# xiaoh/sediFoam

Hardware: AMD Instinct MI355X
Metric: particle-DEM-substeps/sec (higher is better)
Workload: dtype f64; 1 GPU; 1M-particle monodisperse Hertz-history packing (FCC bed, d=1mm, 2% overlap), periodic x/z, wall y, gravity + fix fdrag, 50 DEM sub-steps per step; particles_total=1000188, particles_per_gpu=1000188, neighbor_rebuilds_in_run=140, decomposition=single domain

## Files before the change

### sedifoam_amd/csrc/sf_dem.h

```cpp
#pragma once
#include <map>
#include <string>
#include <vector>
#include <cstdint>
#include <string>
#include <vector>

#include "sf_common.h"
#include "sf_physics.h"

namespace sf {

constexpr int kNeighMask = 0x3FFFFFFF;
constexpr int kTouchBit = 0x40000000;
constexpr int kOwnBit = (int)0x80000000;
constexpr int kIdxBits = 25;
constexpr int kIdxMask = (1 << kIdxBits) - 1;
constexpr int kNoShift = 13;
__host__ __device__ __forceinline__ int neigh_index(int word, int roots)
{
  return roots ? (word & kIdxMask) : (word & kNeighMask);
}
__device__ __forceinline__ void shift_to_image(double4& x, const int word, const double (&prd)[3])
{
// ... 62 lines not shown
constexpr int kBlkMask = (1 << kBlkShift) - 1;
__host__ __device__ inline int* header_vote_ptr(double* slot) { return reinterpret_cast<int*>(slot); }
__host__ __device__ inline int header_vote(const double* slot) { return *reinterpret_cast<const int*>(slot); }

struct DemPtrs {
  const double4* xr_in;
  const double4* vm_in;
  const double4* om_in;
  double4* xr_out;
  double4* vm_out;
  double4* om_out;
  double4* force;
  double4* torque;
  int* neigh;
  int* numneigh;
  const double* shear_in;
  double* shear_out;
  double* fdrag;
  double* DuDt;
  double* vOld;
  double* wshear;
  unsigned char* wtouch;
  const double* xhold;
  const int* mask;
  int* flags;
  const int* sendslot[2];
  double* tx[2];
  double* tx_sendbuf;
  const int* bslot;
  double* const* tx_blkptr;
  const size_t* tx_blkcnt;
  const int* tx_hdr_off;
  int* xcd_time;
  const double* tx_blkshift;
  const struct GsSync* gs_sync;
  int* gs_my_sync;
  int* gs_count;
  const unsigned short* nloc;
  const int* tile_first;
  const int* tile_last;
  const int* stage_start;
  const int* stage_idx;
  const double* mbody;
};

struct GsSync {
  int world, rank;
  long long max_ticks;
  int* my_sync;
  int* peer_sync[32];
};
constexpr int kGsStride = 32;

struct StepParams {
  int nlocal, cap, mode;
  int kstep;
  int nslots;
  int roots;
  double prd[3];
  int part, nb;
  int n_lo, n_hi;
  int trig_test;
  int trig_set;
  int trig_add;
  double margin_sq;
  double dt, trigger_sq;
  GranParams gran;
  CoheParams cohe;
  LubParams lub;
  int nwalls;
  int stage_cap;
  int xcd_remap;
  int xcd_first[8], xcd_count[8];
  int xcd_time;
  WallParams wall[kMaxWalls];
  int have_gravity;
  double gacc[3];
  int have_fdrag;
  double carrier_rho;
  int have_nve;
  int use_groups, nve_bit, grav_bit, fdrag_bit, cohe_bit, freeze_bit;
  int post_freeze;
  int tx_fused, tx_nhdr;
  double tx_lo3[3], tx_hi3[3];
  int gs_on, gs_seq, gs_wait;
  int gs_world, gs_rank;
  int tx_n[2];
  double tx_xlo, tx_xhi, tx_shift[2];
};

struct BinGrid {
  double lo[3], inv[3];
  int n[3];
  int stencil;
  int nbins;
  int tile;
  int nt[3];
  int xslow;
  int wrap[3];
};

__host__ __device__ __forceinline__ int bin_key(const BinGrid& g, int cx, int cy, int cz)
{
  if (g.xslow) return cz + g.n[2] * (cy + g.n[1] * cx);
  if (g.tile <= 1) return cx + g.n[0] * (cy + g.n[1] * cz);
  const int T = g.tile;
  const int tx = cx / T, ty = cy / T, tz = cz / T;
  const int lx = cx - tx * T, ly = cy - ty * T, lz = cz - tz * T;
  return ((tx + g.nt[0] * (ty + g.nt[1] * tz)) * T + lz) * T * T + ly * T + lx;
}

__device__ __forceinline__ int block_sum_int_1024(int v)
{
  __shared__ int ws[16];
  for (int off = 32; off > 0; off >>= 1) v += __shfl_down(v, off, 64);
  const int lane = threadIdx.x & 63, w = threadIdx.x >> 6;
  __syncthreads();
  if (lane == 0) ws[w] = v;
  __syncthreads();
  int t = 0;
  if (threadIdx.x == 0)
    for (int k = 0; k < (int)(blockDim.x >> 6); k++) t += ws[k];
  return t;
}

struct RebuildPredictor {
  long long last = 0;
// ... 384 lines not shown
  LubParams lub_{};
  int nwalls_ = 0;
  WallParams walls_[kMaxWalls];
  WallMotion wall_motion_[kMaxWalls];
  long long wall_time_origin_ = 0;
  long long run_base_step_ = 0;
  bool have_gravity_ = false, have_fdrag_ = false, have_nve_ = false;
  std::map<std::string, int> groups_{{"all", 1}};
  bool use_groups_ = false;
  int nve_bit_ = 1, grav_bit_ = 1, fdrag_bit_ = 1, cohe_bit_ = 1, freeze_bit_ = 0;
  int post_freeze_ = 0;
  int new_group_bit(const std::string& name);
  void mark_frozen();
  double gacc_[3] = {0, 0, 0};
  double carrier_rho_ = 0.0;

  DevArray xr_[2], vm_[2], om_[2], force_, torque_;
  DevArray tag_, type_, mask_, foamCpuId_;
  DevArray fdrag_, DuDt_, vOld_, xhold_;
  DevArray extra_;
  int nextra_ = 0;
  unsigned extra_used_ = 0;
  double extra_init_[8] = {0, 0, 0, 0, 0, 0, 0, 0};
  DevArray wshear_, wtouch_;
  DevArray gsrc_, gshift_;
  DevArray neigh_, numneigh_, shear_[2];
  DevArray neigh_old_, numneigh_old_, ptag_;
  int flags_seq_ = 0;
  bool build_flags_clean_ = false;
  int park_rows_ = 0;
  bool hist_in_place_ = false;
  bool hist_in_place_env_ = true;
  bool build_lds_env_ = true;
  bool rank_permute_env_ = true;
  bool ghost_defer_env_ = true;
  int park_margin_env_ = 8;
  bool build_quad_set_ = false;
  int build_quad_env_ = 0;
  bool build_parks_in_lds() const;
  int hist_buf_ = 0;
  bool hist_single_ = true;
  int hist_mode_env_ = 0;
  bool touch_prefetch_ = true;
  int touch_prefetch_env_ = -1;
  bool touch_first_ = false;
  int touch_first_env_ = -1;
  int opt_lpa_ = 0;
  int opt_ghost_free_ = -1;
  bool ghost_free_ = false;
  int nimages_ = -1;
  bool in_run_ = false;
  RebuildPredictor predict_;
  int nt_policy_ = 2, nt_policy_env_ = -1;
  void measure_list();
  ListStats list_stats() const;
  long long list_sampled_ = 0;
  void choose_kernel();
  DevArray nloc_;
  int* tile_tab_ = nullptr;
  size_t tile_alloc_ = 0;
  int* stage_idx_ = nullptr;
  size_t stage_alloc_ = 0;
  int* eoff_ = nullptr;
  size_t eoff_alloc_ = 0;
  int ntiles_ = 0, stage_cap_ = 0;
  bool lds_active_ = false;
  void build_stage_tables();
  DevArray tmp4_, tmpd_, tmpi_;
  DevArray tmp4b_, tmp4c_, tmpi_b_, tmpi_c_, tmpi_d_, fdrag_alt_, DuDt_alt_, vOld_alt_, extra_alt_, wtouch_alt_;
  DevArray keys_, keys_alt_, perm_, perm_alt_, keys64_, keys64_alt_;
  int* cell_start_ = nullptr;
  size_t cell_alloc_ = 0;
  struct CellRowTables {
    int* own_count;
    int* own_first;
    int* ghost_count;
    int* ghost_first;
  };
  CellRowTables cell_row_tables() const
  {
    return {cell_start_, cell_start_ + cell_alloc_, cell_start_ + 2 * cell_alloc_, cell_start_ + 3 * cell_alloc_};
  }
  struct CellRanges {
    static constexpr int stride = 4;
    int* own_start;
    int* own_end;
    int* ghost_start;
    int* ghost_end;
  };
  CellRanges cell_ranges() const { return {cell_start_, cell_start_ + 1, cell_start_ + 2, cell_start_ + 3}; }
  DevArray hist_perm_;
  bool hist_indirect_ = false;
  bool row_tables_ = false;
  int* image_ = nullptr;
  size_t image_rows_ = 0;
  bool uncounted_wraps_ = false;
  void images_fit();
  int* tagmap_ = nullptr;
  size_t tagmap_alloc_ = 0;
  long long order_version_ = 0, tagmap_builds_ = -1;
  struct IoBuf {
    void* p = nullptr;
    size_t n = 0;
  };
  IoBuf io_d_[3], io_i_[2];
  double* io_doubles(int which, size_t n);
// ... 100 lines not shown
```

### sedifoam_amd/csrc/sf_dem.hip

```cpp
#include "sf_dem.h"

#include <algorithm>
#include <atomic>
#include <chrono>
#include <cmath>
#include <cstdlib>
#include <vector>

#include "sf_dem_dispatch.h"
#include "sf_dem_kernels.h"
#include "sf_dem_rebuild.h"
#include "sf_dem_io.h"
#include "sf_env.h"
#include "sf_dem_lds_kernel.h"
#include "sf_list_policy.h"
#include "sf_rigid.h"
#include "sf_roctx.h"
#include "sf_thermo.h"

namespace sf {

std::string& last_error()
{
  static thread_local std::string e;
// ... 57 lines not shown
    fail("Illegal pair_style command");
  p.kn /= nktv2p;
  p.kt /= nktv2p;
  p.beta = (style == 2 && gamman > 0.0) ? hertz_beta(gamman) : 0.0;
  fold_hertz_constants(p);
}

DemEngine::DemEngine()
{
  int ndev = 0;
  hipError_t e = hipGetDeviceCount(&ndev);
  if (e != hipSuccess || ndev == 0)
    fail("sedifoam_amd: no HIP device available (%s) -- this library has no CPU path",
         e == hipSuccess ? "device count 0" : hipGetErrorString(e));
  SF_HIP(hipStreamCreateWithFlags(&own_stream_, hipStreamNonBlocking));
  stream_ = own_stream_;
  SF_HIP(hipMalloc(&own_flags_, sizeof(int) * F_NFLAGS));
  d_flags_ = own_flags_;
  SF_HIP(hipMalloc(&count64_, sizeof(unsigned long long)));
  SF_HIP(hipHostMalloc(&h_flags_, sizeof(int) * F_NFLAGS));
  memset(h_flags_, 0, sizeof(int) * F_NFLAGS);
  SF_HIP(hipMemsetAsync(d_flags_, 0, sizeof(int) * F_NFLAGS, stream_));
  SF_HIP(hipEventCreate(&ev0_));
  SF_HIP(hipEventCreate(&ev1_));
  SF_HIP(hipEventCreateWithFlags(&ev_flags_, hipEventDisableTiming));
  opt_tile_ = env_int("SF_TILE", opt_tile_);
  opt_xcd_remap_ = env_int("SF_XCD_REMAP", opt_xcd_remap_);
  SF_HIP(hipMalloc(&d_xcd_time_, sizeof(int) * 1024));
  SF_HIP(hipHostMalloc(&h_xcd_time_, sizeof(int) * 1024));
  for (int k = 0; k < 512; k++) h_xcd_time_[512 + k] = (k & 63) == 0 ? INT_MAX : 0;
  SF_HIP(hipMemcpyAsync(d_xcd_time_ + 512, h_xcd_time_ + 512, sizeof(int) * 512, hipMemcpyHostToDevice, stream_));
  xcd_auto_ = env_flag("SF_XCD_BALANCE", xcd_auto_);
  if (const char* e = env_str("SF_XCD_WEIGHTS")) {
    double w[8];
    if (sscanf(e, "%lf,%lf,%lf,%lf,%lf,%lf,%lf,%lf", &w[0], &w[1], &w[2], &w[3], &w[4], &w[5], &w[6], &w[7]) == 8) {
      for (int x = 0; x < 8; x++) xcd_weight_[x] = w[x] > 0.0 ? w[x] : 1.0;
      xcd_weighted_ = true;
      xcd_auto_ = false;
    }
  }
  opt_lds_ = env_int("SF_LDS", opt_lds_);
  roots_ = !opt_lds_;
  if ((opt_sub_env_ = env_override("SF_SUB", opt_sub_))) opt_sub_ = std::max(1, opt_sub_);
  hist_mode_env_ = env_int("SF_HIST_COPIES", hist_mode_env_);
  hist_in_place_env_ = env_flag("SF_HIST_IN_PLACE", hist_in_place_env_);
  build_lds_env_ = env_flag("SF_BUILD_LDS", build_lds_env_);
  rank_permute_env_ = env_flag("SF_RANK_PERMUTE", rank_permute_env_);
  build_quad_set_ = env_override("SF_BUILD_QUAD", build_quad_env_);
  ghost_defer_env_ = env_flag("SF_GHOST_DEFER", ghost_defer_env_);
  park_margin_env_ = env_int("SF_PARK_MARGIN", park_margin_env_);
  touch_prefetch_env_ = env_int("SF_TOUCH_PREFETCH", touch_prefetch_env_);
  touch_first_env_ = env_int("SF_TOUCH_FIRST", touch_first_env_);
  nt_policy_env_ = env_int("SF_NT_POLICY", nt_policy_env_);
  opt_lpa_ = env_int("SF_LPA", opt_lpa_);
  opt_ghost_free_ = env_int("SF_GHOST_FREE", opt_ghost_free_);
  predict_.on = env_flag("SF_QUEUE_PREDICT", predict_.on);
  memset(&gran_, 0, sizeof(gran_));
  memset(&cohe_, 0, sizeof(cohe_));
  memset(&lub_, 0, sizeof(lub_));
  per_atom_ = {&xr_[0], &xr_[1], &vm_[0], &vm_[1], &om_[0], &om_[1], &force_, &torque_, &tag_, &type_,
               &mask_, &foamCpuId_, &fdrag_, &DuDt_, &vOld_, &xhold_, &extra_, &wshear_, &wtouch_, &gsrc_, &gshift_,
               &neigh_, &numneigh_, &shear_[0], &shear_[1], &neigh_old_, &numneigh_old_, &ptag_, &tmp4_,
               &tmpd_, &tmpi_, &keys_, &keys_alt_, &perm_, &perm_alt_, &keys64_, &keys64_alt_,
               &sendlist_[0], &sendlist_[1], &leave_, &nloc_, &isb_, &hist_perm_, &bmask_, &tmp4b_, &tmp4c_,
               &tmpi_b_, &tmpi_c_, &tmpi_d_, &fdrag_alt_, &DuDt_alt_, &vOld_alt_, &extra_alt_, &wtouch_alt_};
}

DemEngine::~DemEngine()
{
  if (stream_) (void)hipStreamSynchronize(stream_);
  rigid_release();
  for (DevArray* a : per_atom_) a->release();
  if (d_blkptr_) (void)hipFree(d_blkptr_);
#ifdef SF_EXP_BUILD_PHASE
  {
    unsigned long long h[8] = {0, 0, 0, 0, 0, 0, 0, 0};
    if (hipMemcpyFromSymbol(h, HIP_SYMBOL(g_build_phase), sizeof(h)) == hipSuccess && (h[0] | h[1] | h[3])) {
      const double tot = (double)(h[0] + h[1] + h[2] + h[3] + h[4] + h[5]);
      fprintf(stderr, "[sedifoam_amd] k_build_neigh wave cycles by phase (%d builds): prologue %.3f  walk %.3f  old tags %.3f  "
              "touch-first pass %.3f  second sweep %.3f  counts %.3f  (sum %.3e cycles)\n", (int)nbuilds_, h[0] / tot, h[1] / tot,
              h[5] / tot, h[2] / tot, h[3] / tot, h[4] / tot, tot);
    }
  }
#endif
  if (thermo_vbuf_) (void)hipFree(thermo_vbuf_);
  if (d_xcd_time_) (void)hipFree(d_xcd_time_);
  if (h_xcd_time_) (void)hipHostFree(h_xcd_time_);
  bslot_.release();
  if (cell_start_) (void)hipFree(cell_start_);
  if (tile_tab_) (void)hipFree(tile_tab_);
  if (bsend_list_) (void)hipFree(bsend_list_);
  if (d_bcount_) (void)hipFree(d_bcount_);
  if (h_bcount_) (void)hipHostFree(h_bcount_);
  if (stage_idx_) (void)hipFree(stage_idx_);
  if (eoff_) (void)hipFree(eoff_);
  if (tagmap_) (void)hipFree(tagmap_);
  if (image_) (void)hipFree(image_);
  for (IoBuf& b : io_d_)
    if (b.p) (void)hipFree(b.p);
  for (IoBuf& b : io_i_)
    if (b.p) (void)hipFree(b.p);
  if (sort_tmp_) (void)hipFree(sort_tmp_);
  if (own_flags_) (void)hipFree(own_flags_);
  if (count64_) (void)hipFree(count64_);
  restart_release();
  if (h_flags_) (void)hipHostFree(h_flags_);
// ... 593 lines not shown
  P.wtouch = wtouch_.as<unsigned char>();
  P.xhold = xhold_.as<double>();
  P.mask = mask_.as<int>();
  P.flags = d_flags_;
  P.nloc = nloc_.as<unsigned short>();
  P.tile_first = tile_tab_;
  for (int f = 0; f < 2; f++) {
    P.sendslot[f] = tx_ready_ ? sendslot_.as<int>() + (size_t)f * sendslot_.cap : nullptr;
    P.tx[f] = tx_ptr_[f];
  }
  P.tx_sendbuf = tx_sendbuf_;
  P.bslot = bslot_.as<int>();
  P.tx_blkptr = d_blkptr_ ? d_blkptr_ + (size_t)tx_par_ * kMaxDirs : nullptr;
  static_assert(sizeof(size_t) == sizeof(double*), "the count row of the block table");
  P.tx_blkcnt = d_blkptr_ ? reinterpret_cast<const size_t*>(d_blkptr_ + 2 * (size_t)kMaxDirs) : nullptr;
  P.tx_hdr_off = tx_hdr_off_;
  P.tx_blkshift = nullptr;
  P.gs_sync = nullptr;
  P.gs_my_sync = nullptr;
  P.gs_count = nullptr;
  P.xcd_time = d_xcd_time_;
  P.tile_last = tile_tab_ ? tile_tab_ + tile_alloc_ : nullptr;
  P.stage_start = tile_tab_ ? tile_tab_ + 3 * tile_alloc_ : nullptr;
  P.stage_idx = stage_idx_;
  P.mbody = rigid_rows_.ptr ? rigid_rows_.as<double>() + (size_t)RR_MBODY * cap_ : nullptr;
  return P;
}

StepParams DemEngine::step_params(int mode, int kstep) const
{
  StepParams S;
  memset(&S, 0, sizeof(S));
  S.nlocal = nlocal_;
  S.cap = (int)cap_;
  S.mode = mode;
  S.kstep = kstep;
  S.nslots = M_;
  S.dt = dt_;
  S.trigger_sq = (0.5 * skin_) * (0.5 * skin_);
  S.roots = roots_ ? 1 : 0;
  for (int k = 0; k < 3; k++) S.prd[k] = boxhi_[k] - boxlo_[k];
  S.part = 0;
  S.nb = 0;
  S.trig_test = F_TRIGGER;
  S.trig_set = F_TRIGGER;
  S.trig_add = 0;
  S.margin_sq = 0.0;
  S.gran = gran_;
  S.cohe = cohe_;
  S.lub = lub_;
  S.nwalls = nwalls_;
  S.xcd_remap = opt_xcd_remap_;
  S.stage_cap = stage_cap_;
  const long long steps = (mode == 2 ? nsteps_ : run_base_step_ + kstep + 1) - wall_time_origin_;
  for (int w = 0; w < nwalls_; w++) {
    WallParams W = walls_[w];
    const WallMotion& M = wall_motion_[w];
    if (M.wiggle) {
      const double om = 2.0 * 3.14159265358979323846 / M.period;
      const double arg = om * (double)steps * dt_;
      if (W.dim == M.axis) {
        W.lo = M.lo0 + M.amplitude - M.amplitude * cos(arg);
        W.hi = M.hi0 + M.amplitude - M.amplitude * cos(arg);
      }
      W.vwall[M.axis] = M.amplitude * om * sin(arg);
    } else if (M.shear) {
      if (W.dim == 3 && M.axis != 2) W.vrot = M.vshear;
      else W.vwall[M.axis] = M.vshear;
    }
    S.wall[w] = W;
  }
  S.have_gravity = have_gravity_;
  for (int k = 0; k < 3; k++) S.gacc[k] = gacc_[k];
  S.have_fdrag = have_fdrag_;
  S.carrier_rho = carrier_rho_;
  S.have_nve = have_nve_;
  S.use_groups = use_groups_ ? 1 : 0;
  S.nve_bit = nve_bit_;
  S.grav_bit = grav_bit_;
  S.fdrag_bit = fdrag_bit_;
  S.cohe_bit = cohe_bit_;
  S.freeze_bit = freeze_bit_;
  S.post_freeze = post_freeze_;
  return S;
}

template <int STYLE, bool COHE, bool LUB, bool GS>
static void launch_plain(int lpa, bool tp, int ntp, dim3 grid, int block, hipStream_t s, const DemPtrs& P,
                         const StepParams& S)
{
  auto go = [&](auto lanes, auto policy) {
    constexpr int LPA = decltype(lanes)::value, NTP = decltype(policy)::value;
    if constexpr (LUB && !COHE) k_substep<STYLE, COHE, LUB, LPA, true, NTP, GS><<<grid, block, 0, s>>>(P, S);
    else if (tp || LUB) k_substep<STYLE, COHE, LUB, LPA, true, NTP, GS><<<grid, block, 0, s>>>(P, S);
    else k_substep<STYLE, COHE, LUB, LPA, false, NTP, GS><<<grid, block, 0, s>>>(P, S);
  };
  if (lpa == 4) go(int_c<4>{}, int_c<0>{});
  else if (lpa == 2) go(int_c<2>{}, int_c<0>{});
  else if (GS || ntp == 0) go(int_c<1>{}, int_c<0>{});
  else if constexpr (!GS) {
    if (ntp == 1) go(int_c<1>{}, int_c<1>{});
    else if (ntp == 3) go(int_c<1>{}, int_c<3>{});
    else go(int_c<1>{}, int_c<2>{});
  }
}

template <int STYLE, bool COHE, bool LUB>
static void launch_lds_one(dim3 grid, size_t lds, hipStream_t s, const DemPtrs& P, const StepParams& S)
{
  static size_t granted = 0;
  if (lds > 65536 && lds > granted) {
    SF_HIP(hipFuncSetAttribute(reinterpret_cast<const void*>(&k_substep_lds<STYLE, COHE, LUB>),
                               hipFuncAttributeMaxDynamicSharedMemorySize, 160 * 1024));
    granted = 160 * 1024;
  }
  static const int threads = env_int("SF_LDS_THREADS", 256);
  k_substep_lds<STYLE, COHE, LUB><<<grid, threads, lds, s>>>(P, S);
}

int DemEngine::lanes_per_atom(int nwork) const
{
  if (opt_lpa_ == 1 || opt_lpa_ == 2 || opt_lpa_ == 4) return opt_lpa_;
  if (nwork < 20 * 1024) return 4;
  if (nwork >= 300 * 1024) return 1;
  static const int slots = [] {
    int dev = 0, cus = 256;
    if (hipGetDevice(&dev) == hipSuccess) (void)hipDeviceGetAttribute(&cus, hipDeviceAttributeMultiprocessorCount, dev);
    return cus * 4 * 3;
  }();
  const double r = (double)nwork / 64.0 / (double)slots;
  if (touch_first_) return 0.5 * std::ceil(2.0 * r) <= std::ceil(r) ? 2 : 1;
  return 0.55 * std::ceil(2.0 * r) < std::ceil(r) ? 2 : 1;
}

void DemEngine::launch_thermo_virial(const DemPtrs& P, const StepParams& S)
{
  if (!thermo_vbuf_) SF_HIP(hipMalloc(&thermo_vbuf_, sizeof(double) * 6 * ::sf::thermo_virial_blocks(INT_MAX)));
  thermo_vblocks_ = ::sf::thermo_virial_blocks(nlocal_);
  thermo_virial_launch(P, S, lub_.enabled != 0, thermo_vbuf_, thermo_vblocks_, stream_);
  thermo_vlaunches_++;
}

void DemEngine::substep_empty_rank(int mode, int kstep, bool gs)
{
  if (thermo_virial_on_ && mode != 0) {
// ... 76 lines not shown
      hipEvent_t e;
      SF_HIP(hipEventCreate(&e));
      prof_ev_.push_back(e);
    }
  }
  if (prof_step_.size() < prof_ev_.size() / 2) prof_step_.resize(prof_ev_.size() / 2);
  prof_step_[prof_used_ / 2] = kstep;
  const hipEvent_t e0 = prof_ev_[prof_used_++], e1 = prof_ev_[prof_used_++];
  SF_HIP(hipEventRecord(e0, stream_));
  prof_open_ = (part == 2);
  return part == 2 ? nullptr : e1;
}

dim3 DemEngine::substep_grid(int mode, int part, StepParams& S, int& block, int& lpa)
{
  const int nwork = part == 2 ? nb_ : (part == 1 ? n_hi_ - n_lo_ : nlocal_);
  if (nwork <= 0) return dim3(0);
  lpa = rigid_ ? 1 : lanes_per_atom(nwork);
  const long long lanes = (long long)nwork * lpa;
  block = block_env() ? block_env() : 64;
  dim3 grid((unsigned)((lanes + block - 1) / block));
  const bool xcd_can = part == 0 && S.xcd_remap == 1 && grid.x >= 2048 && mode == 0;
  if (xcd_can && xcd_auto_ && xcd_countdown_ > 0 && --xcd_countdown_ == 0 && !xcd_sample_pending_) {
    SF_HIP(hipMemcpyAsync(d_xcd_time_, d_xcd_time_ + 512, sizeof(int) * 512, hipMemcpyDeviceToDevice, stream_));
    S.xcd_time = 1;
  }
  if (part == 0 && S.xcd_remap == 1 && xcd_weighted_ && grid.x >= 64) {
    const int nb = (int)grid.x;
    double wsum = 0.0;
    for (int x = 0; x < 8; x++) wsum += xcd_weight_[x];
    int first = 0, most = 0;
    double acc = 0.0;
    for (int x = 0; x < 8; x++) {
      acc += xcd_weight_[x];
      const int end = x == 7 ? nb : std::min(nb, (int)std::llround(nb * acc / wsum));
      S.xcd_first[x] = first;
      S.xcd_count[x] = std::max(0, end - first);
      most = std::max(most, S.xcd_count[x]);
      first = std::max(first, end);
    }
    S.xcd_remap = 2;
    grid = dim3((unsigned)(8 * most));
  }
  stamp_last_grid_ = grid.x;
  return grid;
}

void DemEngine::substep_dispatch(dim3 grid, int block, int lpa, const DemPtrs& P, const StepParams& S)
{
  if (rigid_) return launch_substep_rigid(gran_.style, cohe_.enabled, lub_.enabled, grid, block, stream_, P, S);
  pair_dispatch(gran_.style, cohe_.enabled, lub_.enabled, [&](auto style, auto cohe, auto lub) {
    if (lds_active_) launch_lds_one<style, cohe, lub>(grid, (size_t)stage_cap_ * 88, stream_, P, S);
    else flag_dispatch(S.gs_on != 0, [&](auto gs) {
      launch_plain<style, cohe, lub, gs>(lpa, touch_prefetch_, nt_policy_, grid, block, stream_, P, S);
    });
  });
}

void DemEngine::substep_stamp_record([[maybe_unused]] int mode, [[maybe_unused]] int part)
{
#if SF_EXP_STAMP
  static const char* stamp_file = env_str("SF_STAMP_FILE");
  static const int stamp_at = env_int("SF_STAMP_AT", 60);
  static int stamp_seen = 0;
  static unsigned long long* stamp_buf = nullptr;
  static size_t stamp_blocks = 0, stamp_grid = 0;
  if (stamp_buf && stamp_file && !lds_active_ && part == 0 && mode == 0) stamp_grid = stamp_last_grid_;
  if (stamp_file && !lds_active_ && part == 0 && mode == 0) {
    stamp_seen++;
    if (stamp_seen == stamp_at) {
      const int lpa = lanes_per_atom(nlocal_);
      stamp_blocks = ((size_t)nlocal_ * lpa + 63) / 64 + 8192;
      SF_HIP(hipMalloc(&stamp_buf, sizeof(unsigned long long) * 36 * stamp_blocks));
      SF_HIP(hipMemsetAsync(stamp_buf, 0, sizeof(unsigned long long) * 36 * stamp_blocks, stream_));
      SF_HIP(hipMemcpyToSymbolAsync(HIP_SYMBOL(g_stamp), &stamp_buf, sizeof(stamp_buf), 0, hipMemcpyHostToDevice, stream_));
    } else if (stamp_seen == stamp_at + 1 && stamp_buf) {
      unsigned long long* none = nullptr;
      SF_HIP(hipMemcpyToSymbolAsync(HIP_SYMBOL(g_stamp), &none, sizeof(none), 0, hipMemcpyHostToDevice, stream_));
      std::vector<unsigned long long> h(36 * stamp_blocks);
      SF_HIP(hipMemcpyAsync(h.data(), stamp_buf, sizeof(unsigned long long) * h.size(), hipMemcpyDeviceToHost, stream_));
      SF_HIP(hipStreamSynchronize(stream_));
      if (FILE* f = fopen(stamp_file, "wb")) {
        const unsigned long long g = stamp_grid;
        fwrite(&g, sizeof(g), 1, f);
        fwrite(h.data(), sizeof(unsigned long long), (size_t)36 * stamp_grid, f);
        fclose(f);
      }
      (void)hipFree(stamp_buf);
      stamp_buf = nullptr;
    }
  }
#endif
}

void DemEngine::launch_substep(int in_buf, int mode, int kstep, int part)
{
  const bool gs = gs_ready_ && brick_ && part == 0 && !lds_active_ && mode != 2;
  if (!nlocal_) return substep_empty_rank(mode, kstep, gs);
  if (part == 2 && !nb_) return;
  if (rigid_ && (part || have_subdomain_ || lds_active_ || mode == 0))
    fail("fix rigid/nve needs the whole system on one GPU (one rank, no decomposed domain, no LDS-staged kernel)");
  DemPtrs P = ptrs(in_buf);
  StepParams S = step_params(mode, kstep);
  if (thermo_virial_on_ && mode != 0 && !rigid_ && (part != 1 || !nb_)) launch_thermo_virial(P, S);
  if (gs) substep_ghost_slot_args(P, S);
  if (part) substep_split_args(S, kstep, part);
  substep_forward_pack_args(S, mode, part);
// ... 1197 lines not shown
```

### sedifoam_amd/csrc/sf_dem_kernels.h

```cpp
#pragma once
#include <climits>

#include "sf_dem.h"

#include "sf_dem_variants.h"
#include "sf_dem_gs.h"

namespace sf {

__device__ __forceinline__ Vec3 v3(const double4& a) { return {a.x, a.y, a.z}; }

constexpr bool sf_lean_variant(bool cohe, bool lub, int lpa) { return lpa == 1 && cohe != lub; }

template <bool NT, class T>
__device__ __forceinline__ T ld_stream(const T* p)
{
  if (NT) return __builtin_nontemporal_load(p);
  return *p;
}
template <bool NT, class T>
__device__ __forceinline__ void st_stream(T* p, T v)
{
  if (NT) __builtin_nontemporal_store(v, p);
  else *p = v;
}

__host__ __device__ constexpr bool sf_coop_variant(bool cohe, bool lub, int lpa, bool tp, int ntp)
{
  return lpa == 1 && (ntp == 1 || ntp == 2) && ((cohe && lub) || (!cohe && !lub && !tp));
}
__device__ __forceinline__ void swap32(unsigned& a, unsigned& b)
{
  typedef unsigned sf_u2 __attribute__((ext_vector_type(2)));
  const sf_u2 r = __builtin_amdgcn_permlane32_swap(a, b, false, false);
  a = r.x;
  b = r.y;
}
__device__ __forceinline__ void swap32(double& a, double& b)
{
  unsigned alo = (unsigned)__double2loint(a), ahi = (unsigned)__double2hiint(a);
  unsigned blo = (unsigned)__double2loint(b), bhi = (unsigned)__double2hiint(b);
  swap32(alo, blo);
  swap32(ahi, bhi);
  a = __hiloint2double((int)ahi, (int)alo);
  b = __hiloint2double((int)bhi, (int)blo);
}
__device__ __forceinline__ double4 coop_merge(double4 r)
{
  swap32(r.x, r.z);
  swap32(r.y, r.w);
  return r;
}
__device__ __forceinline__ void coop_indices(const int j, const bool vw, int& ja, int& jb, bool& vwa, bool& vwb)
{
  unsigned a = (unsigned)j | (vw ? 0x80000000u : 0u), b = a;
  swap32(a, b);
  ja = (int)(a & (unsigned)kIdxMask);
  jb = (int)(b & (unsigned)kIdxMask);
  vwa = (int)a < 0;
  vwb = (int)b < 0;
}
__device__ __forceinline__ double4 coop_load(const double4* arr, const int ja, const int jb, const int half,
                                             const bool wa = true, const bool wb = true)
{
  const char* p = reinterpret_cast<const char*>(arr);
  double2 a = {0.0, 0.0}, b = {0.0, 0.0};
  if (wa) a = *reinterpret_cast<const double2*>(p + (((unsigned)ja << 5) | (unsigned)half));
  if (wb) b = *reinterpret_cast<const double2*>(p + (((unsigned)jb << 5) | (unsigned)half));
  return double4{a.x, a.y, b.x, b.y};
}

template <int STYLE, bool COHE, bool LUB, bool LDS, int LPA, bool TP, int NTP, bool GS = false, bool RIGID = false>
__device__ __forceinline__ int substep_particle(const DemPtrs& P, const StepParams& S, const int i, const int q,
                                                 const double4* lx, const double4* lv, const double* lw,
                                                 const unsigned long long gs_w = 0ull, const bool live = true)
{
  constexpr bool COOP = !LDS && sf_coop_variant(COHE, LUB, LPA, TP, NTP);
  const int coop_half = (int)(threadIdx.x & 32) >> 1;
  const size_t cap = (size_t)S.cap;
  const bool shearupdate = (S.mode != 2);
  constexpr int ROOTS = LDS ? 0 : 1;
  constexpr bool NT_LD = NTP != 0, NT_ST = NTP == 1 || NTP == 2, NT_HIST = NTP == 2;
  __builtin_assume(i >= 0 && i < (1 << kIdxBits));

  SF_PH(0);
  bool gs_gated = false;
  if (GS && S.gs_wait && !gs_gated && __ballot(i >= (S.nlocal & ~3))) {
    if (!gs_gate(P.gs_sync, P.flags, S.gs_seq, S.kstep)) return 0;
    gs_gated = true;
  }
  const double4 xi4 = P.xr_in[i];
  const double4 vi4 = P.vm_in[i];
  const double4 wi4 = P.om_in[i];
  const Vec3 xi = v3(xi4), vi = v3(vi4), wi = v3(wi4);
  const double radi = xi4.w, mi = vi4.w;
  double mi_pair = mi;
  if (RIGID) mi_pair = P.mbody[i];

  Vec3 F = {0.0, 0.0, 0.0}, T = {0.0, 0.0, 0.0};
  const int mk = S.use_groups ? P.mask[i] : 1;
  const int nn_all = ld_stream<NT_LD>(&P.numneigh[i]);
  const int nn = COOP ? (live ? nn_all : 0)
                      : LPA == 1 ? nn_all : (nn_all > q ? (nn_all - q + LPA - 1) / LPA : 0);
  const double lub_cutsq = S.lub.cut_global * S.lub.cut_global;

  constexpr bool NEED_VW = (STYLE != 0) || LUB;
  constexpr bool LEAN = sf_lean_variant(COHE, LUB, LPA);
  constexpr bool HIST_PF = !LEAN;
  struct Rec {
    double4 x, v, w;
    Vec3 sh;
    int l;
    bool vw;
  };
  auto load_history = [&](const int jraw, const int slotrow, Vec3& sh) {
    sh = {0.0, 0.0, 0.0};
    if (STYLE == 0 || !(jraw & kTouchBit)) return;
    const bool own = (jraw & kOwnBit) != 0;
    auto ldh = [&](const double* p) { return ld_stream<NT_HIST>(p); };
    if (own) {
      const double* const hin = P.shear_in + (size_t)(3 * slotrow) * cap;
      sh.x = ldh(&hin[i]);
      sh.y = ldh(&(hin + cap)[i]);
      sh.z = ldh(&(hin + 2 * cap)[i]);
    } else {
      const double* src = P.shear_in + (size_t)(3 * ((jraw >> kIdxBits) & 31)) * cap + (size_t)(jraw & kIdxMask);
      sh.x = ldh(src);
      sh.y = ldh(src + cap);
      sh.z = ldh(src + 2 * cap);
      if (LPA > 1) sh = {-sh.x, -sh.y, -sh.z};
    }
  };
  auto wants_vw = [&](const int jraw) {
    return NEED_VW && (LUB || !TP || (jraw & kTouchBit) != 0);
  };
  auto fetch = [&](int jraw, int slotrow, Rec& R) {
// ... 80 lines not shown
    if (STYLE != 0 && LPA == 1 && !own && (jraw & kTouchBit)) sh = {-sh.x, -sh.y, -sh.z};
    jraw_n1 = jraw_n2;
    if (s + 2 < nn) jraw_n2 = ld_stream<NT_LD>(&(nrow + (size_t)(2 * LPA) * cap)[i]);
    else if (COOP) jraw_n2 = 0;
    if (more) fetch(jraw_n1, sl + LPA, nxt);
    double4 xj4 = cur.x, vj4 = cur.v, wj4 = cur.w;
    if (LDS) {
      xj4 = lx[cur.l];
      if (NEED_VW) {
        vj4 = lv[cur.l];
        wj4 = {lw[3 * cur.l], lw[3 * cur.l + 1], lw[3 * cur.l + 2], 0.0};
      }
    }
    if (ROOTS && own) shift_to_image(xj4, jraw, S.prd);
    const Vec3 del = xi - v3(xj4);
    const double rsq = (COOP && s >= nn) ? 1.0e300 : dot(del, del);
    const double radj = xj4.w;
    const double radsum = radi + radj;

    double r_pair = 0.0, rinv_pair = 0.0;
    if (COHE || LUB) sf_sqrt_rsqrt(rsq, r_pair, rinv_pair);
    if (STYLE != 0) {
      if (rsq >= radsum * radsum) {
        if (jraw & kTouchBit) nrow[i] = jraw & ~kTouchBit;
      } else {
        if (!LDS && !cur.vw) {
          vj4 = P.vm_in[cur.l];
          wj4 = P.om_in[cur.l];
        }
        ContactIn c;
        c.del = del;
        c.rsq = rsq;
        if (COHE || LUB) {
          c.r = r_pair;
          c.rinv = rinv_pair;
        } else {
          sf_sqrt_rsqrt(rsq, c.r, c.rinv);
        }
        c.vr = vi - v3(vj4);
        c.wsum = {radi * wi.x + radj * wj4.x, radi * wi.y + radj * wj4.y, radi * wi.z + radj * wj4.z};
        double mj = vj4.w;
        if (RIGID) mj = P.mbody[cur.l];
        const PairScales m = pair_scales(mi_pair, mj, radi, radj, c.r);
        c.overlap = m.overlap;
        c.meff = m.meff;
        c.reff = m.reff;
        if (S.freeze_bit) {
          if (wi4.w != 0.0) c.meff = mj;
          if (wj4.w != 0.0) c.meff = mi_pair;
        }
        ContactOut o;
        gran_history_law<STYLE>(S.gran, S.dt, shearupdate, c, sh, o);
        if (own) {
          st_stream<NT_ST>(&hout[i], sh.x);
          st_stream<NT_ST>(&(hout + cap)[i], sh.y);
          st_stream<NT_ST>(&(hout + 2 * cap)[i], sh.z);
        }
        if (!(jraw & kTouchBit)) nrow[i] = jraw | kTouchBit;
        F = F + o.F;
        T = T - radi * o.tor;
      }
    }
    if (COHE) {
      const double rc = radsum + S.cohe.smax;
      if (S.mode != 2 && (mk & S.cohe_bit) && rsq < rc * rc) {
        const double cc = cohesive_ccel(S.cohe, r_pair, radsum) * rinv_pair;
        F = F + Vec3{del.x * cc, del.y * cc, del.z * cc};
      }
    }
    if (LUB) {
      if (S.lub.flagHI && rsq < lub_cutsq) {
        lubricate_poly_pair(S.lub, del, r_pair, rinv_pair, radi, radj, vi, v3(vj4), wi, v3(wj4), F, T);
      }
    }
    if (more) coop_finish(nxt);
  };
  SF_PH(1);
  int s = 0;
  if constexpr (COOP && !LEAN) {
    for (; s + 1 < nn_wave; s += 2) {
      slot_body(s, RA, RB, true, true);
      slot_body(s + 1, RB, RA, s + 2 < nn_wave, true);
    }
    if (s < nn_wave) slot_body(s, RA, RB, false, true);
  } else if constexpr (COOP) {
    for (; s < nn_wave; s++) {
      slot_body(s, RA, RB, s + 1 < nn_wave, true);
      RA = RB;
    }
  } else if constexpr (!LEAN) {
    for (; s + 1 < nn; s += 2) {
      slot_body(s, RA, RB, true, true);
      slot_body(s + 1, RB, RA, s + 2 < nn, true);
    }
    if (s < nn) slot_body(s, RA, RB, false, false);
  } else {
    for (; s < nn; s++) {
      slot_body(s, RA, RB, s + 1 < nn, true);
      RA = RB;
    }
  }
  SF_PH(27);
  if (COOP && !live) return 1;
  if (LPA > 1) {
    for (int off = 1; off < LPA; off <<= 1) {
      F.x += __shfl_xor(F.x, off, 64); F.y += __shfl_xor(F.y, off, 64); F.z += __shfl_xor(F.z, off, 64);
      T.x += __shfl_xor(T.x, off, 64); T.y += __shfl_xor(T.y, off, 64); T.z += __shfl_xor(T.z, off, 64);
    }
    if (q != 0) return 1;
// ... 137 lines not shown
    for (int k = 0; k < kBrickSlots; k++) {
      const int off = P.bslot[(size_t)k * cap + i];
      if (off < 0) break;
      const int bq = off >> kBlkShift;
      if (GS) {
        const size_t r = (size_t)(off & kBlkMask);
        const double* sh = P.tx_blkshift + 3 * bq;
        gs_store(reinterpret_cast<double4*>(P.tx_blkptr[bq]) + r, xn.x + sh[0], xn.y + sh[1], xn.z + sh[2], radi);
        gs_store(reinterpret_cast<double4*>(P.tx_blkptr[DemEngine::kMaxDirs + bq]) + r, vn.x, vn.y, vn.z, mi);
        gs_store(reinterpret_cast<double4*>(P.tx_blkptr[2 * DemEngine::kMaxDirs + bq]) + r, wn.x, wn.y, wn.z, wi4.w);
        continue;
      }
      double* b = P.tx_blkptr[bq] + (off & kBlkMask);
      const size_t n = P.tx_blkcnt[bq];
      b[0] = xn.x; b[n] = xn.y; b[2 * n] = xn.z;
      b[3 * n] = vn.x; b[4 * n] = vn.y; b[5 * n] = vn.z;
      b[6 * n] = wn.x; b[7 * n] = wn.y; b[8 * n] = wn.z;
    }
  }
  if (S.tx_fused == 1) {
    auto put = [&](double* b, size_t n, double shift) {
      b[0] = xn.x + shift; b[n] = xn.y; b[2 * n] = xn.z;
      b[3 * n] = vn.x; b[4 * n] = vn.y; b[5 * n] = vn.z;
      b[6 * n] = wn.x; b[7 * n] = wn.y; b[8 * n] = wn.z;
    };
    if (txk0 >= 0) put(P.tx[0] + txk0, (size_t)S.tx_n[0], S.tx_shift[0]);
    if (txk1 >= 0) put(P.tx[1] + txk1, (size_t)S.tx_n[1], S.tx_shift[1]);
  }
  SF_PH(29);
  if (RIGID) {
  } else if (LPA == 1 && S.part == 0 && __ballot(1) == ~0ull && (i & 63) == (int)(threadIdx.x & 63)) {
    const int lane = threadIdx.x & 63;
    const int base = i - lane;
    auto store_shuffled = [&](double4* arr, double a0, double a1, double a2, double a3) {
      swap32(a0, a2);
      swap32(a1, a3);
      char* dst = reinterpret_cast<char*>(arr + base) + ((lane & 31) << 5) + ((lane & 32) >> 1);
      *reinterpret_cast<double2*>(dst) = double2{a0, a1};
      *reinterpret_cast<double2*>(dst + 1024) = double2{a2, a3};
    };
    store_shuffled(P.xr_out, xn.x, xn.y, xn.z, radi);
    store_shuffled(P.vm_out, vn.x, vn.y, vn.z, mi);
    store_shuffled(P.om_out, wn.x, wn.y, wn.z, wi4.w);
  } else {
    P.xr_out[i] = {xn.x, xn.y, xn.z, radi};
    P.vm_out[i] = {vn.x, vn.y, vn.z, mi};
    P.om_out[i] = {wn.x, wn.y, wn.z, wi4.w};
  }
  if (S.mode != 0) {
    P.force[i] = {F.x, F.y, F.z, 0.0};
    P.torque[i] = {T.x, T.y, T.z, 0.0};
  }
  SF_PH(30);
  return 1 | (txb ? 2 : 0) | (gs_trig ? 4 : 0);
}

#define SF_SUBSTEP_ATTR __attribute__((amdgpu_waves_per_eu((COHE || LUB) && !sf_lean_variant(COHE, LUB, LPA) ? 1 : 3)))
__device__ __forceinline__ int xcd_contiguous_block()
{
  const int bid = blockIdx.x, nb = gridDim.x, xcd = bid & 7, q = nb >> 3, r = nb & 7;
  return (xcd < r ? xcd * (q + 1) : r * (q + 1) + (xcd - r) * q) + (bid >> 3);
}

template <int STYLE, bool COHE, bool LUB, int LPA, bool TP, int NTP, bool GS = false, bool RIGID = false>
__global__ __launch_bounds__(256) SF_SUBSTEP_ATTR void k_substep(DemPtrs P, StepParams S)
{
  if (__atomic_load_n(&P.flags[S.trig_test], __ATOMIC_RELAXED) < S.kstep) return;
  if (GS && __atomic_load_n(&P.flags[F_HALO_TIMEOUT], __ATOMIC_RELAXED) != 0) return;
  SF_STAMP_WORKGROUP();
  int bid = blockIdx.x;
  int gs_expected = 0;
  bool gs_poller = false;
  if (S.xcd_remap == 2) {
    const int xcd = bid & 7, loc = bid >> 3;
    if (loc >= S.xcd_count[xcd]) return;
    bid = S.xcd_first[xcd] + loc;
    if (GS) {
      const int lx = (int)(threadIdx.x & 7);
      gs_expected = S.xcd_count[lx];
      int firstx = 0;
      while (firstx < 7 && S.xcd_count[firstx] == 0) firstx++;
      gs_poller = loc == 0 && xcd == firstx;
    }
  } else {
    const int nb = gridDim.x, xcd = bid & 7, q = nb >> 3, r = nb & 7, loc = bid >> 3;
    if (S.xcd_remap) bid = (xcd < r ? xcd * (q + 1) : r * (q + 1) + (xcd - r) * q) + loc;
    if (GS) {
      const int lx = (int)(threadIdx.x & 7);
      gs_expected = lx < r ? q + 1 : q;
      gs_poller = blockIdx.x == 0;
    }
  }
  unsigned long long gs_w = gs_word(S.gs_seq, INT_MAX);
  if (GS && S.gs_wait) {
    const int r = (int)(threadIdx.x & 63);
    if (r < S.gs_world && r != S.gs_rank) gs_w = gs_read_line(P.gs_my_sync + kGsStride * r);
  }
  const int tid = bid * blockDim.x + threadIdx.x;
  int i = tid / LPA;
  const int q = tid % LPA;
  constexpr bool COOPK = sf_coop_variant(COHE, LUB, LPA, TP, NTP);
  bool live = true;
  if (S.part == 2) {
    live = i < S.nb;
    if (live && i >= S.n_lo) i += S.n_hi - S.n_lo;
  } else if (S.part == 1) {
    i += S.n_lo;
    live = i < S.n_hi;
  } else {
    live = i < S.nlocal;
  }
  if (!live) i = 0;
  if (!GS && !(COOPK ? __ballot(live) != 0 : live)) return;
  const int xq = (int)(blockIdx.x & 7) * 64;
  if (S.xcd_time && threadIdx.x == 0 && (blockIdx.x >> 3) == 0) atomicMin(&P.xcd_time[xq], (int)(wall_clock64() & 0x3fffffff));
  if (GS) {
    int ran = 1;
    if (COOPK ? __ballot(live) != 0 : live)
      ran = substep_particle<STYLE, COHE, LUB, false, LPA, TP, NTP, true>(P, S, i, q, nullptr, nullptr, nullptr, gs_w, live);
    if (__ballot(ran == 0)) return;
    if (S.mode == 0) gs_done(P, S, (ran & 2) != 0, (ran & 4) != 0, gs_poller, gs_expected);
  } else {
    substep_particle<STYLE, COHE, LUB, false, LPA, TP, NTP, false, RIGID>(P, S, i, q, nullptr, nullptr, nullptr, 0ull, live);
  }
  if (S.xcd_time && threadIdx.x == 0 && ((blockIdx.x >> 3) & 7) == 0)
    atomicMax(&P.xcd_time[xq + 32], (int)(wall_clock64() & 0x3fffffff));
}


__global__ __launch_bounds__(256) static void k_initial_integrate(double4* xr, double4* vm, double4* om,
                                                           const double4* force, const double4* torque,
                                                           const double* xhold, int* flags, int nlocal,
                                                           size_t cap, double dt, double trigger_sq,
                                                           const int* mask, int nve_bit)
{
  const int i = blockIdx.x * blockDim.x + threadIdx.x;
  if (i >= nlocal) return;
  if (mask && !(mask[i] & nve_bit)) return;
  double4 x = xr[i], v = vm[i], w = om[i];
  const double4 f = force[i], t = torque[i];
  const double dtf = 0.5 * dt;
  const double dtfm = dtf / v.w;
  const double dtirot = (dtf / 0.4) / (x.w * x.w * v.w);
  v.x += dtfm * f.x;
  v.y += dtfm * f.y;
  v.z += dtfm * f.z;
  x.x += dt * v.x;
  x.y += dt * v.y;
  x.z += dt * v.z;
  w.x += dtirot * t.x;
  w.y += dtirot * t.y;
  w.z += dtirot * t.z;
  xr[i] = x;
  vm[i] = v;
  om[i] = w;
  const double dx = x.x - xhold[i], dy = x.y - xhold[cap + i], dz = x.z - xhold[2 * cap + i];
  if (dx * dx + dy * dy + dz * dz > trigger_sq) atomicMin(flags, -1);
}

__global__ __launch_bounds__(256) static void k_ghost_forward(double4* xr, double4* vm, double4* om,
                                                       const int* gsrc, const double* gshift,
                                                       int nlocal, int nghost, size_t cap,
                                                       const int* flags, int kstep, int trig_word, int phase)
{
  if (__atomic_load_n(&flags[trig_word], __ATOMIC_RELAXED) < kstep) return;
  const int k = blockIdx.x * blockDim.x + threadIdx.x;
  if (k >= nghost) return;
  const int g = nlocal + k;
  const int src = gsrc[g];
  if (src < 0) return;
  if (phase == 1 && src >= nlocal) return;
  if (phase == 2 && src < nlocal) return;
  double4 x = xr[src];
  x.x += gshift[g];
  x.y += gshift[cap + g];
  x.z += gshift[2 * cap + g];
// ... 34 lines not shown
```

Before: 4.469 billion particle-substeps/s.

## Park contact-history stores in LDS and flush after particle update

Adds a parked kernel variant that buffers up to eight per-contact shear-history triples in shared memory during the contact loop, instead of streaming them straight to global memory. After the integration and force stores, it flushes the buffered entries to the history arrays with a wave-uniform loop. The aim is to take history writes out of the latency-critical contact loop and batch them at the end. The cost is dynamic LDS per block (8×3×64 doubles per wave), which can lower occupancy, plus extra bookkeeping registers.

```diff
diff --git a/sedifoam_amd/csrc/sf_dem.h b/sedifoam_amd/csrc/sf_dem.h
--- a/sedifoam_amd/csrc/sf_dem.h
+++ b/sedifoam_amd/csrc/sf_dem.h
@@ -138,6 +138,8 @@
 };
 constexpr int kGsStride = 32;
 
+constexpr int kParkEntries = 8;
+
 struct StepParams {
   int nlocal, cap, mode;
   int kstep;
@@ -159,6 +161,7 @@
   int xcd_remap;
   int xcd_first[8], xcd_count[8];
   int xcd_time;
+  int park_entries;
   WallParams wall[kMaxWalls];
   int have_gravity;
   double gacc[3];
@@ -649,6 +652,8 @@
   bool in_run_ = false;
   RebuildPredictor predict_;
   int nt_policy_ = 2, nt_policy_env_ = -1;
+  bool park_hist_ = true;
+  int park_entries_ = kParkEntries;
   void measure_list();
   ListStats list_stats() const;
   long long list_sampled_ = 0;
diff --git a/sedifoam_amd/csrc/sf_dem.hip b/sedifoam_amd/csrc/sf_dem.hip
--- a/sedifoam_amd/csrc/sf_dem.hip
+++ b/sedifoam_amd/csrc/sf_dem.hip
@@ -133,6 +133,8 @@
   touch_prefetch_env_ = env_int("SF_TOUCH_PREFETCH", touch_prefetch_env_);
   touch_first_env_ = env_int("SF_TOUCH_FIRST", touch_first_env_);
   nt_policy_env_ = env_int("SF_NT_POLICY", nt_policy_env_);
+  park_hist_ = env_flag("SF_PARK_HIST", park_hist_);
+  park_entries_ = std::min(kParkEntries, std::max(1, env_int("SF_PARK_ENTRIES", park_entries_)));
   opt_lpa_ = env_int("SF_LPA", opt_lpa_);
   opt_ghost_free_ = env_int("SF_GHOST_FREE", opt_ghost_free_);
   predict_.on = env_flag("SF_QUEUE_PREDICT", predict_.on);
@@ -832,6 +834,7 @@
   S.nwalls = nwalls_;
   S.xcd_remap = opt_xcd_remap_;
   S.stage_cap = stage_cap_;
+  S.park_entries = park_entries_;
   const long long steps = (mode == 2 ? nsteps_ : run_base_step_ + kstep + 1) - wall_time_origin_;
   for (int w = 0; w < nwalls_; w++) {
     WallParams W = walls_[w];
@@ -866,11 +869,18 @@
 }
 
 template <int STYLE, bool COHE, bool LUB, bool GS>
-static void launch_plain(int lpa, bool tp, int ntp, dim3 grid, int block, hipStream_t s, const DemPtrs& P,
+static void launch_plain(int lpa, bool tp, int ntp, bool park, dim3 grid, int block, hipStream_t s, const DemPtrs& P,
                          const StepParams& S)
 {
   auto go = [&](auto lanes, auto policy) {
     constexpr int LPA = decltype(lanes)::value, NTP = decltype(policy)::value;
+    if constexpr (sf_park_variant(STYLE, COHE, LUB, false, LPA, true, GS, false)) {
+      if (park && tp) {
+        const size_t lds = (size_t)((block + 63) / 64) * kParkWaveDoubles * sizeof(double);
+        k_substep<STYLE, COHE, LUB, LPA, true, NTP, GS, false, true><<<grid, block, lds, s>>>(P, S);
+        return;
+      }
+    }
     if constexpr (LUB && !COHE) k_substep<STYLE, COHE, LUB, LPA, true, NTP, GS><<<grid, block, 0, s>>>(P, S);
     else if (tp || LUB) k_substep<STYLE, COHE, LUB, LPA, true, NTP, GS><<<grid, block, 0, s>>>(P, S);
     else k_substep<STYLE, COHE, LUB, LPA, false, NTP, GS><<<grid, block, 0, s>>>(P, S);
@@ -1053,7 +1063,7 @@
   pair_dispatch(gran_.style, cohe_.enabled, lub_.enabled, [&](auto style, auto cohe, auto lub) {
     if (lds_active_) launch_lds_one<style, cohe, lub>(grid, (size_t)stage_cap_ * 88, stream_, P, S);
     else flag_dispatch(S.gs_on != 0, [&](auto gs) {
-      launch_plain<style, cohe, lub, gs>(lpa, touch_prefetch_, nt_policy_, grid, block, stream_, P, S);
+      launch_plain<style, cohe, lub, gs>(lpa, touch_prefetch_, nt_policy_, park_hist_, grid, block, stream_, P, S);
     });
   });
 }
diff --git a/sedifoam_amd/csrc/sf_dem_kernels.h b/sedifoam_amd/csrc/sf_dem_kernels.h
--- a/sedifoam_amd/csrc/sf_dem_kernels.h
+++ b/sedifoam_amd/csrc/sf_dem_kernels.h
@@ -28,6 +28,11 @@
 __host__ __device__ constexpr bool sf_coop_variant(bool cohe, bool lub, int lpa, bool tp, int ntp)
 {
   return lpa == 1 && (ntp == 1 || ntp == 2) && ((cohe && lub) || (!cohe && !lub && !tp));
+}
+constexpr int kParkWaveDoubles = kParkEntries * 3 * 64;
+__host__ __device__ constexpr bool sf_park_variant(int style, bool cohe, bool lub, bool lds, int lpa, bool tp, bool gs, bool rigid)
+{
+  return style != 0 && !cohe && !lub && !lds && lpa == 1 && tp && !gs && !rigid;
 }
 __device__ __forceinline__ void swap32(unsigned& a, unsigned& b)
 {
@@ -70,7 +75,8 @@
   return double4{a.x, a.y, b.x, b.y};
 }
 
-template <int STYLE, bool COHE, bool LUB, bool LDS, int LPA, bool TP, int NTP, bool GS = false, bool RIGID = false>
+template <int STYLE, bool COHE, bool LUB, bool LDS, int LPA, bool TP, int NTP, bool GS = false, bool RIGID = false,
+          bool PARK = false>
 __device__ __forceinline__ int substep_particle(const DemPtrs& P, const StepParams& S, const int i, const int q,
                                                  const double4* lx, const double4* lv, const double* lw,
                                                  const unsigned long long gs_w = 0ull, const bool live = true)
@@ -82,6 +88,15 @@
   constexpr int ROOTS = LDS ? 0 : 1;
   constexpr bool NT_LD = NTP != 0, NT_ST = NTP == 1 || NTP == 2, NT_HIST = NTP == 2;
   __builtin_assume(i >= 0 && i < (1 << kIdxBits));
+  static_assert(!PARK || sf_park_variant(STYLE, COHE, LUB, LDS, LPA, TP, GS, RIGID), "no parked form of this kernel");
+  extern __shared__ double sf_park_area[];
+  auto park_top = [&]() {
+    return (unsigned)(((int)(threadIdx.x >> 6) * kParkWaveDoubles + (int)(threadIdx.x & 63) + S.park_entries * (3 * 64)) * 8);
+  };
+  auto park_at = [&](const unsigned byte) { return reinterpret_cast<double*>(reinterpret_cast<char*>(sf_park_area) + byte); };
+  constexpr unsigned kParkStep = (1u << 20) + 3 * 64 * 8;
+  unsigned park_mask = 0, park_state = 0;
+  if constexpr (PARK) park_state = ((unsigned)S.park_entries << 20) | park_top();
 
   SF_PH(0);
   bool gs_gated = false;
@@ -268,9 +283,18 @@
         ContactOut o;
         gran_history_law<STYLE>(S.gran, S.dt, shearupdate, c, sh, o);
         if (own) {
-          st_stream<NT_ST>(&hout[i], sh.x);
-          st_stream<NT_ST>(&(hout + cap)[i], sh.y);
-          st_stream<NT_ST>(&(hout + 2 * cap)[i], sh.z);
+          if (PARK && park_state >= (1u << 20) && sl < 32) {
+            park_state -= kParkStep;
+            double* const pk = park_at(park_state & 0xfffffu);
+            pk[0] = sh.x;
+            pk[64] = sh.y;
+            pk[128] = sh.z;
+            park_mask |= 1u << sl;
+          } else {
+            st_stream<NT_ST>(&hout[i], sh.x);
+            st_stream<NT_ST>(&(hout + cap)[i], sh.y);
+            st_stream<NT_ST>(&(hout + 2 * cap)[i], sh.z);
+          }
         }
         if (!(jraw & kTouchBit)) nrow[i] = jraw | kTouchBit;
         F = F + o.F;
@@ -514,6 +538,19 @@
     P.torque[i] = {T.x, T.y, T.z, 0.0};
   }
   SF_PH(30);
+  if constexpr (PARK) {
+    unsigned at = park_top();
+    for (int sl = 0; sl < 32 && __ballot((park_mask >> sl) != 0); sl++) {
+      if ((park_mask >> sl) & 1u) {
+        at -= 3 * 64 * 8;
+        const double* const pk = park_at(at);
+        double* const hout = P.shear_out + (size_t)(3 * sl) * cap;
+        st_stream<NT_ST>(&hout[i], pk[0]);
+        st_stream<NT_ST>(&(hout + cap)[i], pk[64]);
+        st_stream<NT_ST>(&(hout + 2 * cap)[i], pk[128]);
+      }
+    }
+  }
   return 1 | (txb ? 2 : 0) | (gs_trig ? 4 : 0);
 }
 
@@ -524,7 +561,7 @@
   return (xcd < r ? xcd * (q + 1) : r * (q + 1) + (xcd - r) * q) + (bid >> 3);
 }
 
-template <int STYLE, bool COHE, bool LUB, int LPA, bool TP, int NTP, bool GS = false, bool RIGID = false>
+template <int STYLE, bool COHE, bool LUB, int LPA, bool TP, int NTP, bool GS = false, bool RIGID = false, bool PARK = false>
 __global__ __launch_bounds__(256) SF_SUBSTEP_ATTR void k_substep(DemPtrs P, StepParams S)
 {
   if (__atomic_load_n(&P.flags[S.trig_test], __ATOMIC_RELAXED) < S.kstep) return;
@@ -583,7 +620,7 @@
     if (__ballot(ran == 0)) return;
     if (S.mode == 0) gs_done(P, S, (ran & 2) != 0, (ran & 4) != 0, gs_poller, gs_expected);
   } else {
-    substep_particle<STYLE, COHE, LUB, false, LPA, TP, NTP, false, RIGID>(P, S, i, q, nullptr, nullptr, nullptr, 0ull, live);
+    substep_particle<STYLE, COHE, LUB, false, LPA, TP, NTP, false, RIGID, PARK>(P, S, i, q, nullptr, nullptr, nullptr, 0ull, live);
   }
   if (S.xcd_time && threadIdx.x == 0 && ((blockIdx.x >> 3) & 7) == 0)
     atomicMax(&P.xcd_time[xq + 32], (int)(wall_clock64() & 0x3fffffff));
```

Result: no change. 4.440 billion particle-substeps/s (-0.7%).
